# RemcoHoger/Space-Filling-Curves-for-Vision-Transformers

Measured on AMD Instinct MI355X. Metric: images/sec ViT-B/16 224px Hilbert-order training, higher is better.
Workload: dtype bf16; 1 GPU; vit_b16_224_hilbert: 224x224 Hilbert pixel order, 16x16-pixel tokens, batch 256/GPU, full train step (fwd+CE+bwd+clip+AdamW); global_batch=256, parallelism=dp1, hip_graph=False

## Files before the change

space-filling-curves-for-vision-transformers_amd/csrc/gemm8p.hip:

```cpp
#include "common_host.h"
#include "gemm_core.h"
#include <mutex>
#include <type_traits>
#include <unordered_map>

namespace sfcvit {
namespace {

using namespace gemm_core;

namespace p8 {

constexpr int T = 512, HALF = 16384, KTB = 65536, LDS_BYTES = 2 * KTB;
constexpr int LDS_TQ = LDS_BYTES, LDS_PATCH = LDS_TQ + 64, LDS_BIAS = LDS_PATCH + 8 * 2048, LDS_MAX = P8_LDS_MAX;
static_assert(LDS_BIAS == P8_LDS_BIAS, "dispatch.h prices the bias vector at this offset");
enum { RELU = P8_RELU, DROP = P8_DROP, RES = P8_RES, DACT = P8_DACT, CSUM = P8_CSUM, BITS = P8_BITS };

typedef const __attribute__((address_space(1))) void *gptr_t;
typedef __attribute__((address_space(3))) void *lptr_t;

template <int N> __device__ __forceinline__ void wait_vm() { asm volatile("s_waitcnt vmcnt(%0)" ::"n"(N) : "memory"); }
template <int N> __device__ __forceinline__ void wait_lgkm() {
    asm volatile("s_waitcnt lgkmcnt(%0)" ::"n"(N) : "memory");
    __builtin_amdgcn_sched_barrier(0);
}
__device__ __forceinline__ void bar() {
    __builtin_amdgcn_sched_barrier(0);
    __builtin_amdgcn_s_barrier();
    __builtin_amdgcn_sched_barrier(0);
}

struct Cursor {
    int tile, k0;
    const uint16_t *p;
};

struct StoreMap {
    int wa;
    int ra;
    long coff;
};

template <int MASK>
__device__ __forceinline__ void epilogue_math(const sfcvit_gemm_args &g, int m, int n, float (&v)[16], const float (&bv)[16],
                                              const u32x4 (&side)[2], uint32_t thresh, float keep_scale, float dact_scale,
                                              uint32_t rk_in0, uint32_t rk_in1, u32x4 &w0, u32x4 &w1) {
    if (!(MASK & DACT)) {
#pragma unroll
        for (int r = 0; r < 16; r++) v[r] += bv[r];
    }
    if (MASK & RELU) {
#pragma unroll
        for (int r = 0; r < 16; r++) v[r] = fmaxf(v[r], 0.f);
    }
    if (MASK & DROP) {
        const uint64_t row = uint64_t(m) + uint64_t(uint32_t(g.row_offset));
        const uint32_t rk = mix32(uint32_t(row) * 0x9E3779B1u + ((row >> 32) ? rk_in1 : rk_in0));
#pragma unroll
        for (int p = 0; p < 8; p++) {
            bool k0, k1;
            drop_keep2(rk, uint32_t(n >> 1) + p, thresh, k0, k1);
            v[2 * p] = k0 ? v[2 * p] * keep_scale : 0.f;
            v[2 * p + 1] = k1 ? v[2 * p + 1] * keep_scale : 0.f;
        }
    }
    if (MASK & RES) {
        float rv[16];
        unpack8f(side[0], rv);
        unpack8f(side[1], rv + 8);
#pragma unroll
        for (int r = 0; r < 16; r++) v[r] += rv[r];
    }
    if ((MASK & BITS) && (MASK & RELU)) {
        uint32_t bits = 0;
#pragma unroll
        for (int r = 0; r < 16; r++) bits |= uint32_t(v[r] > 0.f) << r;
        uint8_t *mp = static_cast<uint8_t *>(g.actmask) + size_t(m) * g.ld_actmask + (n >> 3);
        asm volatile("global_store_short %0, %1, off\n\ts_nop 1" ::"v"(mp), "v"(bits) : "memory");
    }
    if (MASK & DACT) {
        if (MASK & BITS) {
            const uint32_t bits = side[0][0];
#pragma unroll
            for (int r = 0; r < 16; r++) v[r] = (bits >> r & 1u) ? v[r] * dact_scale : 0.f;
        } else {
            float a[16];
            unpack8f(side[0], a);
            unpack8f(side[1], a + 8);
#pragma unroll
            for (int r = 0; r < 16; r++) v[r] = a[r] > 0.f ? v[r] * dact_scale : 0.f;
        }
    }
    w0 = u32x4{pack2bf(v[0], v[1]), pack2bf(v[2], v[3]), pack2bf(v[4], v[5]), pack2bf(v[6], v[7])};
    w1 = u32x4{pack2bf(v[8], v[9]), pack2bf(v[10], v[11]), pack2bf(v[12], v[13]), pack2bf(v[14], v[15])};
}

#define SFCVIT_XROW(a, b) "ds_write_b128 %[wa], " a "\n\tds_write_b128 %[wb], " b "\n\tds_read_b128 " a ", %[ra]\n\tds_read_b128 " b ", %[ra] offset:1024\n\t"
template <int NR>
__device__ __forceinline__ void patch_exchange(u32x4 (&w)[NR][2], const StoreMap &sm) {
    static_assert(NR >= 1 && NR <= 8, "rows per batch");
    const int wa = sm.wa, wb = sm.wa ^ 16, ra = sm.ra;
    if constexpr (NR == 8)
        asm volatile(SFCVIT_XROW("%0", "%1") SFCVIT_XROW("%2", "%3") SFCVIT_XROW("%4", "%5") SFCVIT_XROW("%6", "%7")
                     SFCVIT_XROW("%8", "%9") SFCVIT_XROW("%10", "%11") SFCVIT_XROW("%12", "%13") SFCVIT_XROW("%14", "%15") "s_waitcnt lgkmcnt(0)"
                     : "+v"(w[0][0]), "+v"(w[0][1]), "+v"(w[1][0]), "+v"(w[1][1]), "+v"(w[2][0]), "+v"(w[2][1]), "+v"(w[3][0]), "+v"(w[3][1]),
                       "+v"(w[4][0]), "+v"(w[4][1]), "+v"(w[5][0]), "+v"(w[5][1]), "+v"(w[6][0]), "+v"(w[6][1]), "+v"(w[7][0]), "+v"(w[7][1])
                     : [wa] "v"(wa), [wb] "v"(wb), [ra] "v"(ra) : "memory");
    else if constexpr (NR == 7)
        asm volatile(SFCVIT_XROW("%0", "%1") SFCVIT_XROW("%2", "%3") SFCVIT_XROW("%4", "%5") SFCVIT_XROW("%6", "%7")
                     SFCVIT_XROW("%8", "%9") SFCVIT_XROW("%10", "%11") SFCVIT_XROW("%12", "%13") "s_waitcnt lgkmcnt(0)"
                     : "+v"(w[0][0]), "+v"(w[0][1]), "+v"(w[1][0]), "+v"(w[1][1]), "+v"(w[2][0]), "+v"(w[2][1]), "+v"(w[3][0]), "+v"(w[3][1]),
                       "+v"(w[4][0]), "+v"(w[4][1]), "+v"(w[5][0]), "+v"(w[5][1]), "+v"(w[6][0]), "+v"(w[6][1])
                     : [wa] "v"(wa), [wb] "v"(wb), [ra] "v"(ra) : "memory");
    else if constexpr (NR == 6)
        asm volatile(SFCVIT_XROW("%0", "%1") SFCVIT_XROW("%2", "%3") SFCVIT_XROW("%4", "%5") SFCVIT_XROW("%6", "%7")
                     SFCVIT_XROW("%8", "%9") SFCVIT_XROW("%10", "%11") "s_waitcnt lgkmcnt(0)"
                     : "+v"(w[0][0]), "+v"(w[0][1]), "+v"(w[1][0]), "+v"(w[1][1]), "+v"(w[2][0]), "+v"(w[2][1]), "+v"(w[3][0]), "+v"(w[3][1]),
                       "+v"(w[4][0]), "+v"(w[4][1]), "+v"(w[5][0]), "+v"(w[5][1])
                     : [wa] "v"(wa), [wb] "v"(wb), [ra] "v"(ra) : "memory");
    else if constexpr (NR == 4)
        asm volatile(SFCVIT_XROW("%0", "%1") SFCVIT_XROW("%2", "%3") SFCVIT_XROW("%4", "%5") SFCVIT_XROW("%6", "%7") "s_waitcnt lgkmcnt(0)"
                     : "+v"(w[0][0]), "+v"(w[0][1]), "+v"(w[1][0]), "+v"(w[1][1]), "+v"(w[2][0]), "+v"(w[2][1]), "+v"(w[3][0]), "+v"(w[3][1])
                     : [wa] "v"(wa), [wb] "v"(wb), [ra] "v"(ra) : "memory");
    else
        static_assert(NR == 8, "patch_exchange: batch sizes 4, 6, 7, 8");
}
#undef SFCVIT_XROW

__device__ __forceinline__ void store_row_pair(const sfcvit_gemm_args &g, int m, int n, const StoreMap &sm, const u32x4 &w0, const u32x4 &w1) {
    uint16_t *c = static_cast<uint16_t *>(g.c) + size_t(m) * g.ldc + n + sm.coff;
    asm volatile("global_store_dwordx4 %0, %1, off sc0 sc1 nt\n\ts_nop 1" ::"v"(c), "v"(w0) : "memory");
    asm volatile("global_store_dwordx4 %0, %1, off sc0 sc1 nt\n\ts_nop 1" ::"v"(c + size_t(8) * g.ldc), "v"(w1) : "memory");
}


template <int NI, int MASK, bool P2 = false>
__global__ __launch_bounds__(T) void gemm8p_kernel(const sfcvit_gemm_args g, unsigned *__restrict__ counters, int stag_slots, int stag_ticks, int walk) {
    constexpr int BM = 32 * NI, GR = 16 * NI;
    extern __shared__ __attribute__((aligned(16))) char smem[];
    if (stag_ticks > 0) {
        const uint64_t until = __builtin_amdgcn_s_memrealtime() + uint64_t((blockIdx.x >> 3) % stag_slots) * uint64_t(stag_ticks);
        while (__builtin_amdgcn_s_memrealtime() < until) __builtin_amdgcn_s_sleep(8);
    }
    const int tid = threadIdx.x, lane = tid & 63, wid = __builtin_amdgcn_readfirstlane(tid >> 6), wr = wid >> 2, wc = wid & 3;
    const int q = lane >> 4, nl = lane & 15;
    const int K = g.K, NT = g.N / 256, ntiles = ((g.M + BM - 1) / BM) * NT, KT = K / 64, m_last = g.M - BM;
    const uint16_t *A = static_cast<const uint16_t *>(g.a);
    const uint16_t *B = static_cast<const uint16_t *>(g.b);
    const int G = gridDim.x, per_xcd = G >> 3, xcd = blockIdx.x & 7;
    int *const tq = reinterpret_cast<int *>(smem + LDS_TQ);
    auto tile_of = [&](unsigned l) __attribute__((always_inline)) {
        const long t = long(l / unsigned(per_xcd)) * G + xcd * per_xcd + int(l % unsigned(per_xcd));
        if (t >= ntiles) return -1;
        if (walk > 0 && walk < NT) {
            const unsigned MT = unsigned(ntiles / NT), full = unsigned(NT / walk) * MT * unsigned(walk), ut = unsigned(t);
            const unsigned wcur = ut < full ? unsigned(walk) : unsigned(NT % walk), base = ut < full ? (ut / (MT * walk)) * walk : unsigned(NT / walk) * walk;
            const unsigned tt = ut < full ? ut % (MT * walk) : ut - full;
            return int((tt / wcur) << 16 | (base + tt % wcur));
        }
        return int((unsigned(t) / unsigned(NT)) << 16 | (unsigned(t) % unsigned(NT)));
    };
    auto finish = [&]() __attribute__((always_inline)) {
        if (tid == 0) {
            const unsigned old = atomicAdd(counters + 8, 1u);
            if (old == unsigned(G) - 1u) {
#pragma unroll
                for (int i = 0; i < 9; i++) counters[i] = 0u;
            }
        }
    };
    if (tid == 0) {
        const unsigned l0 = atomicAdd(counters + xcd, 1u);
        tq[0] = tile_of(l0);
        const unsigned l1 = atomicAdd(counters + xcd, 1u);
        tq[1] = tile_of(l1);
    }
    const bool has_bias = !(MASK & DACT) && g.bias != nullptr;
    if (has_bias)
        for (int i = tid; i < g.N / 8; i += T)
            *reinterpret_cast<u32x4 *>(smem + LDS_BIAS + i * 16) = static_cast<const u32x4 *>(g.bias)[i];
    __syncthreads();

    int tile_cur = __builtin_amdgcn_readfirstlane(tq[0]);
    if (tile_cur < 0) { finish(); return; }
    unsigned drawn = 0;
    if (tid == 0) drawn = atomicAdd(counters + xcd, 1u);
    const int tile_first = tile_cur;
    int t = 0;

    const int r1 = 8 * wid + (lane >> 3);
    const int sc = (lane & 7) ^ ((r1 >> 1) & 7);
    const int w1 = (r1 < GR - 64) ? r1 : r1 - (NI == 7 ? 16 : 32);
    const int b_row = (r1 >> 5) * 64 + ((r1 & 15) >> 2) * 16 + ((r1 >> 4) & 1) * 4 + (r1 & 3);
    const uint32_t voffA0 = (uint32_t(r1) * uint32_t(g.lda) + sc * 8) * 2, voffA1 = (uint32_t(64 + w1) * uint32_t(g.lda) + sc * 8) * 2;
    const uint32_t voffB = (uint32_t(b_row) * uint32_t(g.ldb) + sc * 8) * 2;
    const size_t a_second = size_t(GR) * g.lda, b_second = size_t(128) * g.ldb, b_h1 = size_t(8) * g.ldb;

    auto cursor_at = [&](int seq, int tile, bool is_a) __attribute__((always_inline)) {
        Cursor c;
        c.tile = seq;
        c.k0 = 0;
        if (tile < 0) tile = tile_first;
        c.p = is_a ? A + size_t(min((tile >> 16) * BM, m_last)) * g.lda : B + size_t(tile & 0xFFFF) * 256 * g.ldb;
        return c;
    };
    const uint16_t *next_a = nullptr, *next_b = nullptr;
    auto set_next = [&](int seq) __attribute__((always_inline)) {
        const Cursor na = cursor_at(seq, __builtin_amdgcn_readfirstlane(tq[seq & 3]), true);
        const Cursor nb = cursor_at(seq, __builtin_amdgcn_readfirstlane(tq[seq & 3]), false);
        next_a = na.p;
        next_b = nb.p;
    };
    auto advance = [&](Cursor &c, bool is_a) __attribute__((always_inline)) {
        if (c.k0 + 64 == K) { c.tile++; c.k0 = 0; c.p = is_a ? next_a : next_b; }
        else { c.k0 += 64; c.p += 64; }
    };
    const int m0_wave = wid * 1024;
    auto dma16 = [&](const uint16_t *base, uint32_t voff, int lds) __attribute__((always_inline)) {
        asm volatile("s_mov_b32 m0, %2\n\ts_nop 0\n\tglobal_load_lds_dwordx4 %0, %1"
                     :
                     : "v"(voff), "s"(base), "s"(lds)
                     : "memory");
    };
    auto stage_a = [&](const Cursor &c, int buf, int h) __attribute__((always_inline)) {
        const int d = m0_wave + buf * KTB + h * HALF;
        const uint32_t vo = h ? voffA1 : voffA0;
        dma16(c.p, vo, d);
        dma16(c.p + a_second, vo, d + 8192);
    };
    auto stage_b = [&](const Cursor &c, int buf, int h) __attribute__((always_inline)) {
        const uint16_t *p = c.p + (h ? b_h1 : 0);
        const int d = m0_wave + buf * KTB + 2 * HALF + h * HALF;
        dma16(p, voffB, d);
        dma16(p + b_second, voffB, d + 8192);
    };

    const int o0 = nl * 128 + ((q ^ ((nl >> 1) & 7)) << 4);
    const int a_off0 = wr * 8192 + o0, a_off1 = wr * 8192 + (o0 ^ 64);
    const int b_off0 = 2 * HALF + wc * 4096 + o0, b_off1 = 2 * HALF + wc * 4096 + (o0 ^ 64);
    bf16x8 fa0[4][2], fa1[NI - 4][2], fb0[2][2], fb1[2][2];
    auto read_a0 = [&](int buf) __attribute__((always_inline)) {
#pragma unroll
        for (int i = 0; i < 4; i++) {
            fa0[i][0] = *reinterpret_cast<const bf16x8 *>(smem + a_off0 + buf * KTB + i * 2048);
            fa0[i][1] = *reinterpret_cast<const bf16x8 *>(smem + a_off1 + buf * KTB + i * 2048);
        }
    };
    auto read_a1 = [&](int buf) __attribute__((always_inline)) {
#pragma unroll
        for (int i = 0; i < NI - 4; i++) {
            fa1[i][0] = *reinterpret_cast<const bf16x8 *>(smem + a_off0 + buf * KTB + HALF + i * 2048);
            fa1[i][1] = *reinterpret_cast<const bf16x8 *>(smem + a_off1 + buf * KTB + HALF + i * 2048);
        }
    };
    auto read_b = [&](bf16x8 (&fb)[2][2], int buf, int sub) __attribute__((always_inline)) {
#pragma unroll
        for (int j = 0; j < 2; j++) {
            fb[j][0] = *reinterpret_cast<const bf16x8 *>(smem + b_off0 + buf * KTB + sub * HALF + j * 2048);
            fb[j][1] = *reinterpret_cast<const bf16x8 *>(smem + b_off1 + buf * KTB + sub * HALF + j * 2048);
        }
    };

    f32x4 acc[NI][4];
    auto zero_acc = [&]() __attribute__((always_inline)) {
#pragma unroll
        for (int i = 0; i < NI; i++)
#pragma unroll
            for (int j = 0; j < 4; j++) acc[i][j] = f32x4{0.f, 0.f, 0.f, 0.f};
    };
    auto mma0 = [&](const bf16x8 (&fb)[2][2], int bsub) __attribute__((always_inline)) {
        __builtin_amdgcn_s_setprio(1);
#pragma unroll
        for (int kk = 0; kk < 2; kk++)
#pragma unroll
            for (int i = 0; i < 4; i++)
#pragma unroll
                for (int j = 0; j < 2; j++)
                    acc[i][bsub * 2 + j] = __builtin_amdgcn_mfma_f32_16x16x32_bf16(fb[j][kk], fa0[i][kk], acc[i][bsub * 2 + j], 0, 0, 0);
        __builtin_amdgcn_s_setprio(0);
    };
    auto mma1 = [&](const bf16x8 (&fb)[2][2], int bsub) __attribute__((always_inline)) {
        __builtin_amdgcn_s_setprio(1);
#pragma unroll
        for (int kk = 0; kk < 2; kk++)
#pragma unroll
            for (int i = 0; i < NI - 4; i++)
#pragma unroll
                for (int j = 0; j < 2; j++)
                    acc[4 + i][bsub * 2 + j] = __builtin_amdgcn_mfma_f32_16x16x32_bf16(fb[j][kk], fa1[i][kk], acc[4 + i][bsub * 2 + j], 0, 0, 0);
        __builtin_amdgcn_s_setprio(0);
    };

    const uint32_t thresh = (MASK & DROP) ? drop_thresh(g.dropout_p) : 0u;
    const float keep_scale = (MASK & DROP) ? 1.f / (1.f - g.dropout_p) : 1.f;
    const uint32_t seed_e = (MASK & DROP) ? eff_seed(g.dropout_seed, g.seed_off) : 0u;
    const uint32_t rk_in0 = (MASK & DROP) ? mix32(seed_e) : 0u, rk_in1 = (MASK & DROP) ? mix32(seed_e ^ 0x7FEB352Du) : 0u;
    const float dact_scale = g.dact_scale != 0.f ? g.dact_scale : 1.f;
    auto draw = [&]() __attribute__((always_inline)) {
        if (tid == 0) {
            tq[(t + 2) & 3] = tile_of(drawn);
            drawn = atomicAdd(counters + xcd, 1u);
        }
    };
    auto epilogue = [&]() __attribute__((always_inline)) {
        const int tile = tile_cur;
        int te = tid;
        asm volatile("" : "+v"(te));
        const int le = te & 63, qe = le >> 4, ne = le & 15;
        StoreMap sm;
        {
            const int patch = LDS_PATCH + wid * 2048, r0 = le >> 3, ch = le & 7;
            sm.wa = patch + ne * 128 + (((2 * qe) ^ (ne & 7)) << 4);
            sm.ra = patch + r0 * 128 + ((ch ^ r0) << 4);
            sm.coff = long(r0 - ne) * g.ldc + (8 * ch - 16 * qe);
        }
        const int m_new = (tile >> 16) * BM;
        const int m0 = min(m_new, m_last) + wr * GR + ne, n0 = (tile & 0xFFFF) * 256 + wc * 64 + qe * 16;
        mfma_fence();
        float bv[16];
        if (has_bias) {
            const char *bp = smem + LDS_BIAS + n0 * 2;
            unpack8f(*reinterpret_cast<const u32x4 *>(bp), bv);
            unpack8f(*reinterpret_cast<const u32x4 *>(bp + 16), bv + 8);
        } else {
#pragma unroll
            for (int r = 0; r < 16; r++) bv[r] = 0.f;
        }
        const uint16_t *sp = (MASK & RES) ? static_cast<const uint16_t *>(g.residual) : static_cast<const uint16_t *>(g.aux_in);
        const size_t ld_side = (MASK & RES) ? size_t(g.ldr) : size_t(g.ldaux);
        float cs[16];
#pragma unroll
        for (int r = 0; r < 16; r++) cs[r] = 0.f;
        auto batch = [&](auto i0c, auto i1c) __attribute__((always_inline)) {
            constexpr int i0 = decltype(i0c)::value, i1 = decltype(i1c)::value;
            u32x4 side[i1 - i0][2];
            if ((MASK & DACT) && (MASK & BITS)) {
#pragma unroll
                for (int i = i0; i < i1; i++)
                    side[i - i0][0][0] = *reinterpret_cast<const uint16_t *>(static_cast<const uint8_t *>(g.actmask) +
                                                                             size_t(m0 + 16 * i) * g.ld_actmask + (n0 >> 3));
            } else if (MASK & (RES | DACT)) {
#pragma unroll
                for (int i = i0; i < i1; i++) {
                    const uint16_t *p = sp + size_t(m0 + 16 * i) * ld_side + n0;
                    side[i - i0][0] = *reinterpret_cast<const u32x4 *>(p);
                    side[i - i0][1] = *reinterpret_cast<const u32x4 *>(p + 8);
                }
            }
            u32x4 pk[i1 - i0][2];
            static_for<i0, i1>([&](auto ic) __attribute__((always_inline)) {
                constexpr int i = decltype(ic)::value;
                float v[16] = {acc[i][0][0], acc[i][0][1], acc[i][0][2], acc[i][0][3], acc[i][1][0], acc[i][1][1],
                               acc[i][1][2], acc[i][1][3], acc[i][2][0], acc[i][2][1], acc[i][2][2], acc[i][2][3],
                               acc[i][3][0], acc[i][3][1], acc[i][3][2], acc[i][3][3]};
                epilogue_math<MASK>(g, m0 + 16 * i, n0, v, bv, side[i - i0], thresh, keep_scale, dact_scale, rk_in0, rk_in1,
                                    pk[i - i0][0], pk[i - i0][1]);
                if (MASK & CSUM) {
                    const bool own = m0 + 16 * i >= m_new;
#pragma unroll
                    for (int r = 0; r < 16; r++) cs[r] += own ? v[r] : 0.f;
                }
            });
            patch_exchange<i1 - i0>(pk, sm);
            static_for<i0, i1>([&](auto ic) __attribute__((always_inline)) {
                constexpr int i = decltype(ic)::value;
                store_row_pair(g, m0 + 16 * i, n0, sm, pk[i - i0][0], pk[i - i0][1]);
            });
        };
        if constexpr (NI == 8 && ((MASK & (DROP | RES)) == (DROP | RES) || (MASK & (DACT | CSUM | BITS)) == (DACT | CSUM))) {
            batch(std::integral_constant<int, 0>{}, std::integral_constant<int, 4>{});
            batch(std::integral_constant<int, 4>{}, std::integral_constant<int, NI>{});
        } else {
            batch(std::integral_constant<int, 0>{}, std::integral_constant<int, NI>{});
        }
        if (MASK & CSUM) {
#pragma unroll
            for (int r = 0; r < 16; r++) cs[r] = row16_sum(cs[r]);
            if (ne == 0) {
                float *pp = static_cast<float *>(g.workspace) + size_t(2 * (tile >> 16) + wr) * g.N + n0;
#pragma unroll
                for (int r4 = 0; r4 < 4; r4++)
                    *reinterpret_cast<f32x4 *>(pp + 4 * r4) = f32x4{cs[4 * r4], cs[4 * r4 + 1], cs[4 * r4 + 2], cs[4 * r4 + 3]};
            }
        }
        zero_acc();
    };

    Cursor ca = cursor_at(0, tile_cur, true), cb = cursor_at(0, tile_cur, false);
    stage_b(cb, 0, 0); stage_a(ca, 0, 0); stage_a(ca, 0, 1); stage_b(cb, 0, 1);
    advance(ca, true);
    advance(cb, false);
    if (P2) {
        stage_b(cb, 1, 0); stage_a(ca, 1, 0); stage_b(cb, 1, 1);
        advance(cb, false);
        wait_vm<6>();
    } else {
        stage_b(cb, 1, 0); stage_a(ca, 1, 0); stage_a(ca, 1, 1); stage_b(cb, 1, 1);
        advance(ca, true);
        advance(cb, false);
        wait_vm<8>();
    }
    bar();
    if (wr == 1) bar();
    zero_acc();

    constexpr int NSTORE = 2 * NI + ((MASK & CSUM) ? 4 : 0) + (((MASK & BITS) && (MASK & RELU)) ? NI : 0);
    auto stage_next = [&](int buf) __attribute__((always_inline)) {
        stage_a(ca, buf, 1);
        advance(ca, true);
        stage_b(cb, buf, 1);
        advance(cb, false);
        __builtin_amdgcn_sched_barrier(0);
    };
    auto ktile = [&](int buf, bool first, bool last) __attribute__((always_inline)) {
        read_b(fb0, buf, 0);
        read_a0(buf);
        bar();
        wait_lgkm<0>();
        mma0(fb0, 0);
        bar();
        read_a1(buf);
        bar();
        wait_lgkm<0>();
        mma1(fb0, 0);
        if (first) set_next(t + 1);
        bar();
        read_b(fb1, buf, 1);
        stage_b(cb, buf, 0);
        bar();
        wait_lgkm<0>();
        mma1(fb1, 1);
        bar();
        stage_a(ca, buf, 0);
        if (first && t > 0) wait_vm<4 + NSTORE>();
        else wait_vm<4>();
        bar();
        mma0(fb1, 1);
        if (last) {
            if (wr == 0) {
                bar();
                draw();
            }
            stage_next(buf);
            epilogue();
            if (wr == 1) bar();
        } else {
            bar();
            stage_next(buf);
        }
    };
    auto ktile2 = [&](int buf, bool first, bool last) __attribute__((always_inline)) {
        read_b(fb0, buf, 0);
        read_b(fb1, buf, 1);
        read_a0(buf);
        stage_a(ca, buf ^ 1, 1);
        advance(ca, true);
        __builtin_amdgcn_sched_barrier(0);
        if (first && t > 0) wait_vm<8 + NSTORE>();
        else wait_vm<8>();
        wait_lgkm<0>();
        bar();
        mma0(fb0, 0);
        mma0(fb1, 1);
        if (first) set_next(t + 1);
        bar();
        read_a1(buf);
        stage_b(cb, buf, 0);
        stage_a(ca, buf, 0);
        stage_b(cb, buf, 1);
        advance(cb, false);
        __builtin_amdgcn_sched_barrier(0);
        if (first && t > 0) wait_vm<8 + NSTORE>();
        else wait_vm<8>();
        wait_lgkm<0>();
        bar();
        mma1(fb0, 0);
        mma1(fb1, 1);
        if (last) {
            if (wr == 0) {
                bar();
                draw();
            }
            epilogue();
            if (wr == 1) bar();
        } else {
            bar();
        }
    };
    int kt = 0;
    for (;;) {
        if (P2) ktile2(0, kt == 0, false);
        else ktile(0, kt == 0, false);
        kt += 2;
        const bool last = kt == KT;
        if (P2) ktile2(1, false, last);
        else ktile(1, false, last);
        if (last) {
            kt = 0;
            t++;
            tile_cur = __builtin_amdgcn_readfirstlane(tq[t & 3]);
            if (tile_cur < 0) break;
        }
    }
    if (wr == 0) bar();
    wait_vm<0>();
    finish();
}


template <bool P2>
__global__ __launch_bounds__(T) void gemm8p_km_kernel(const sfcvit_gemm_args g, int kt_per_split, int nsplits) {
    extern __shared__ __attribute__((aligned(16))) char smem[];
    const int tid = threadIdx.x, lane = tid & 63, wid = tid >> 6, wr = wid >> 2, wc = wid & 3;
    const int q4 = lane >> 4, nl = lane & 15;
    const int NT = g.N / 256, KT = g.K / 64;
    const int tiles = (g.M / 256) * NT;
    const int unit = (blockIdx.x & 7) * (gridDim.x >> 3) + (blockIdx.x >> 3);
    if (unit >= tiles * nsplits) return;
    const int tile = unit % tiles, z = unit / tiles;
    const int m0 = (tile / NT) * 256, n0 = (tile % NT) * 256;
    const int kt_beg = z * kt_per_split;
    const int nkt = min(kt_per_split, KT - kt_beg);
    const uint16_t *A = static_cast<const uint16_t *>(g.a) + size_t(kt_beg) * 64 * g.lda + m0;
    const uint16_t *B = static_cast<const uint16_t *>(g.b) + size_t(kt_beg) * 64 * g.ldb + n0;

    const int kr = 4 * wid + (lane >> 4);
    const int sw = (kr & 3) | (((kr >> 3) & 1) << 2);
    const int c16 = ((((lane & 15) >> 1) ^ sw) << 1) | (lane & 1);
    const size_t offA = size_t(kr) * g.lda + c16 * 8, offB = size_t(kr) * g.ldb + c16 * 8;
    const size_t a32 = size_t(32) * g.lda, b32 = size_t(32) * g.ldb, a64 = size_t(64) * g.lda, b64 = size_t(64) * g.ldb;
    char *const lds_piece = smem + tid * 16;
    const uint16_t *ca = A, *cb = B;
    int akt = 0, bkt = 0;
    auto advance_a = [&]() __attribute__((always_inline)) {
        if (++akt < nkt) ca += a64;
    };
    auto advance_b = [&]() __attribute__((always_inline)) {
        if (++bkt < nkt) cb += b64;
    };
    auto stage_a = [&](int buf, int h) __attribute__((always_inline)) {
        const uint16_t *p = ca + offA + h * 128;
        char *d = lds_piece + buf * KTB + h * HALF;
        __builtin_amdgcn_global_load_lds((gptr_t)p, (lptr_t)d, 16, 0, 0);
        __builtin_amdgcn_global_load_lds((gptr_t)(p + a32), (lptr_t)(d + 8192), 16, 0, 0);
    };
    auto stage_b = [&](int buf, int h) __attribute__((always_inline)) {
        const uint16_t *p = cb + offB + h * 128;
        char *d = lds_piece + buf * KTB + 2 * HALF + h * HALF;
        __builtin_amdgcn_global_load_lds((gptr_t)p, (lptr_t)d, 16, 0, 0);
        __builtin_amdgcn_global_load_lds((gptr_t)(p + b32), (lptr_t)(d + 8192), 16, 0, 0);
    };

    const int qq = nl >> 2, pp = nl & 3;
    const int lane_sw = qq | ((q4 & 1) << 2);
    const int row_off = (8 * q4 + qq) * 256 + 8 * pp;
    int a_addr[8], b_addr[4];
#pragma unroll
    for (int i = 0; i < 8; i++)
        a_addr[i] = (i >> 2) * HALF + row_off + (((wr * 4 + (i & 3)) ^ lane_sw) << 5);
#pragma unroll
    for (int j = 0; j < 4; j++)
        b_addr[j] = 2 * HALF + (j >> 1) * HALF + row_off + (((wc * 2 + (j & 1)) ^ lane_sw) << 5);
#define SFCVIT_TR(dst, addr, off) asm volatile("ds_read_b64_tr_b16 %0, %1 offset:" #off : "=v"(dst) : "v"(addr) : "memory")
    auto tr_frag2 = [&](bf16x8 (&f)[2], int addr) __attribute__((always_inline)) {
        bf16x4 l0, h0, l1, h1;
        SFCVIT_TR(l0, addr, 0);
        SFCVIT_TR(h0, addr, 1024);
        SFCVIT_TR(l1, addr, 8192);
        SFCVIT_TR(h1, addr, 9216);
        f[0] = __builtin_shufflevector(l0, h0, 0, 1, 2, 3, 4, 5, 6, 7);
        f[1] = __builtin_shufflevector(l1, h1, 0, 1, 2, 3, 4, 5, 6, 7);
    };
    bf16x8 fa0[4][2], fa1[4][2], fb0[2][2], fb1[2][2];
    auto read_a2 = [&](bf16x8 (&fa)[4][2], int sub, int i0) __attribute__((always_inline)) {
#pragma unroll
        for (int i = i0; i < i0 + 2; i++) tr_frag2(fa[i], a_addr[sub * 4 + i]);
    };
    auto read_b = [&](bf16x8 (&fb)[2][2], int sub) __attribute__((always_inline)) {
#pragma unroll
        for (int j = 0; j < 2; j++) tr_frag2(fb[j], b_addr[sub * 2 + j]);
    };
    auto flip = [&]() __attribute__((always_inline)) {
#pragma unroll
        for (int i = 0; i < 8; i++) a_addr[i] ^= KTB;
#pragma unroll
        for (int j = 0; j < 4; j++) b_addr[j] ^= KTB;
    };

    f32x4 acc[8][4];
#pragma unroll
    for (int i = 0; i < 8; i++)
#pragma unroll
        for (int j = 0; j < 4; j++) acc[i][j] = f32x4{0.f, 0.f, 0.f, 0.f};
    auto mma = [&](const bf16x8 (&fa)[4][2], const bf16x8 (&fb)[2][2], int asub, int bsub) __attribute__((always_inline)) {
        __builtin_amdgcn_s_setprio(1);
#pragma unroll
        for (int kk = 0; kk < 2; kk++)
#pragma unroll
            for (int i = 0; i < 4; i++)
#pragma unroll
                for (int j = 0; j < 2; j++)
                    acc[asub * 4 + i][bsub * 2 + j] =
                        __builtin_amdgcn_mfma_f32_16x16x32_bf16(fb[j][kk], fa[i][kk], acc[asub * 4 + i][bsub * 2 + j], 0, 0, 0);
        __builtin_amdgcn_s_setprio(0);
    };

    if (P2) {
        stage_b(0, 0); stage_a(0, 0); stage_a(0, 1); stage_b(0, 1);
        advance_a();
        advance_b();
        stage_b(1, 0); stage_a(1, 0); stage_b(1, 1);
        advance_b();
        wait_vm<6>();
        bar();
        if (wr == 1) bar();
        auto ktile2 = [&](int buf) __attribute__((always_inline)) {
            read_b(fb0, 0);
            read_b(fb1, 1);
            read_a2(fa0, 0, 0);
            read_a2(fa0, 0, 2);
            stage_a(buf ^ 1, 1);
            advance_a();
            wait_vm<8>();
            wait_lgkm<0>();
            bar();
            mma(fa0, fb0, 0, 0);
            mma(fa0, fb1, 0, 1);
            bar();
            read_a2(fa1, 1, 0);
            read_a2(fa1, 1, 2);
            stage_b(buf, 0);
            stage_a(buf, 0);
            stage_b(buf, 1);
            advance_b();
            wait_vm<8>();
            wait_lgkm<0>();
            bar();
            mma(fa1, fb0, 1, 0);
            mma(fa1, fb1, 1, 1);
            bar();
            flip();
        };
        for (int k = 0; k < nkt; k += 2) {
            ktile2(0);
            ktile2(1);
        }
    } else {
        stage_b(0, 0); stage_a(0, 0); stage_a(0, 1); stage_b(0, 1);
        advance_a();
// ... 144 lines not shown
```

Baseline: 8260 images/s.

## Trim register pressure and scalar bookkeeping in persistent GEMM kernel

Drops the per-cursor tile and k0 counters and replaces the K-boundary test in advance with a wrap flag computed in the outer loop. Lane-dependent constants are recomputed after the epilogue, and empty asm barriers keep leading dimensions and scheduling values in SGPRs, to lower VGPR pressure in the heavy DROP|RES variant. Accumulator zeroing is overlapped with the LDS patch exchange by splitting the wait out of patch_exchange. The aim is to avoid spills and cut scalar and vector overhead in the main loop, at the cost of fragile compiler-steering asm and some recomputation.

```diff
diff --git a/space-filling-curves-for-vision-transformers_amd/csrc/gemm8p.hip b/space-filling-curves-for-vision-transformers_amd/csrc/gemm8p.hip
--- a/space-filling-curves-for-vision-transformers_amd/csrc/gemm8p.hip
+++ b/space-filling-curves-for-vision-transformers_amd/csrc/gemm8p.hip
@@ -31,7 +31,6 @@
 }
 
 struct Cursor {
-    int tile, k0;
     const uint16_t *p;
 };
 
@@ -42,7 +41,7 @@
 };
 
 template <int MASK>
-__device__ __forceinline__ void epilogue_math(const sfcvit_gemm_args &g, int m, int n, float (&v)[16], const float (&bv)[16],
+__device__ __forceinline__ void epilogue_math(const sfcvit_gemm_args &g, int ld_bits, int m, int n, float (&v)[16], const float (&bv)[16],
                                               const u32x4 (&side)[2], uint32_t thresh, float keep_scale, float dact_scale,
                                               uint32_t rk_in0, uint32_t rk_in1, u32x4 &w0, u32x4 &w1) {
     if (!(MASK & DACT)) {
@@ -75,7 +74,7 @@
         uint32_t bits = 0;
 #pragma unroll
         for (int r = 0; r < 16; r++) bits |= uint32_t(v[r] > 0.f) << r;
-        uint8_t *mp = static_cast<uint8_t *>(g.actmask) + size_t(m) * g.ld_actmask + (n >> 3);
+        uint8_t *mp = static_cast<uint8_t *>(g.actmask) + size_t(m) * ld_bits + (n >> 3);
         asm volatile("global_store_short %0, %1, off\n\ts_nop 1" ::"v"(mp), "v"(bits) : "memory");
     }
     if (MASK & DACT) {
@@ -96,72 +95,102 @@
 }
 
 #define SFCVIT_XROW(a, b) "ds_write_b128 %[wa], " a "\n\tds_write_b128 %[wb], " b "\n\tds_read_b128 " a ", %[ra]\n\tds_read_b128 " b ", %[ra] offset:1024\n\t"
+#define SFCVIT_W4 "+v"(w[0][0]), "+v"(w[0][1]), "+v"(w[1][0]), "+v"(w[1][1]), "+v"(w[2][0]), "+v"(w[2][1]), "+v"(w[3][0]), "+v"(w[3][1])
+#define SFCVIT_W6 SFCVIT_W4, "+v"(w[4][0]), "+v"(w[4][1]), "+v"(w[5][0]), "+v"(w[5][1])
+#define SFCVIT_W7 SFCVIT_W6, "+v"(w[6][0]), "+v"(w[6][1])
+#define SFCVIT_W8 SFCVIT_W7, "+v"(w[7][0]), "+v"(w[7][1])
+#define SFCVIT_X4 SFCVIT_XROW("%0", "%1") SFCVIT_XROW("%2", "%3") SFCVIT_XROW("%4", "%5") SFCVIT_XROW("%6", "%7")
+#define SFCVIT_X6 SFCVIT_X4 SFCVIT_XROW("%8", "%9") SFCVIT_XROW("%10", "%11")
+#define SFCVIT_X7 SFCVIT_X6 SFCVIT_XROW("%12", "%13")
+#define SFCVIT_X8 SFCVIT_X7 SFCVIT_XROW("%14", "%15")
 template <int NR>
 __device__ __forceinline__ void patch_exchange(u32x4 (&w)[NR][2], const StoreMap &sm) {
-    static_assert(NR >= 1 && NR <= 8, "rows per batch");
+    static_assert(NR == 4 || NR == 6 || NR == 7 || NR == 8, "patch_exchange: batch sizes 4, 6, 7, 8");
     const int wa = sm.wa, wb = sm.wa ^ 16, ra = sm.ra;
-    if constexpr (NR == 8)
-        asm volatile(SFCVIT_XROW("%0", "%1") SFCVIT_XROW("%2", "%3") SFCVIT_XROW("%4", "%5") SFCVIT_XROW("%6", "%7")
-                     SFCVIT_XROW("%8", "%9") SFCVIT_XROW("%10", "%11") SFCVIT_XROW("%12", "%13") SFCVIT_XROW("%14", "%15") "s_waitcnt lgkmcnt(0)"
-                     : "+v"(w[0][0]), "+v"(w[0][1]), "+v"(w[1][0]), "+v"(w[1][1]), "+v"(w[2][0]), "+v"(w[2][1]), "+v"(w[3][0]), "+v"(w[3][1]),
-                       "+v"(w[4][0]), "+v"(w[4][1]), "+v"(w[5][0]), "+v"(w[5][1]), "+v"(w[6][0]), "+v"(w[6][1]), "+v"(w[7][0]), "+v"(w[7][1])
-                     : [wa] "v"(wa), [wb] "v"(wb), [ra] "v"(ra) : "memory");
-    else if constexpr (NR == 7)
-        asm volatile(SFCVIT_XROW("%0", "%1") SFCVIT_XROW("%2", "%3") SFCVIT_XROW("%4", "%5") SFCVIT_XROW("%6", "%7")
-                     SFCVIT_XROW("%8", "%9") SFCVIT_XROW("%10", "%11") SFCVIT_XROW("%12", "%13") "s_waitcnt lgkmcnt(0)"
-                     : "+v"(w[0][0]), "+v"(w[0][1]), "+v"(w[1][0]), "+v"(w[1][1]), "+v"(w[2][0]), "+v"(w[2][1]), "+v"(w[3][0]), "+v"(w[3][1]),
-                       "+v"(w[4][0]), "+v"(w[4][1]), "+v"(w[5][0]), "+v"(w[5][1]), "+v"(w[6][0]), "+v"(w[6][1])
-                     : [wa] "v"(wa), [wb] "v"(wb), [ra] "v"(ra) : "memory");
-    else if constexpr (NR == 6)
-        asm volatile(SFCVIT_XROW("%0", "%1") SFCVIT_XROW("%2", "%3") SFCVIT_XROW("%4", "%5") SFCVIT_XROW("%6", "%7")
-                     SFCVIT_XROW("%8", "%9") SFCVIT_XROW("%10", "%11") "s_waitcnt lgkmcnt(0)"
-                     : "+v"(w[0][0]), "+v"(w[0][1]), "+v"(w[1][0]), "+v"(w[1][1]), "+v"(w[2][0]), "+v"(w[2][1]), "+v"(w[3][0]), "+v"(w[3][1]),
-                       "+v"(w[4][0]), "+v"(w[4][1]), "+v"(w[5][0]), "+v"(w[5][1])
-                     : [wa] "v"(wa), [wb] "v"(wb), [ra] "v"(ra) : "memory");
-    else if constexpr (NR == 4)
-        asm volatile(SFCVIT_XROW("%0", "%1") SFCVIT_XROW("%2", "%3") SFCVIT_XROW("%4", "%5") SFCVIT_XROW("%6", "%7") "s_waitcnt lgkmcnt(0)"
-                     : "+v"(w[0][0]), "+v"(w[0][1]), "+v"(w[1][0]), "+v"(w[1][1]), "+v"(w[2][0]), "+v"(w[2][1]), "+v"(w[3][0]), "+v"(w[3][1])
-                     : [wa] "v"(wa), [wb] "v"(wb), [ra] "v"(ra) : "memory");
-    else
-        static_assert(NR == 8, "patch_exchange: batch sizes 4, 6, 7, 8");
-}
+    if constexpr (NR == 8) asm volatile(SFCVIT_X8 : SFCVIT_W8 : [wa] "v"(wa), [wb] "v"(wb), [ra] "v"(ra) : "memory");
+    else if constexpr (NR == 7) asm volatile(SFCVIT_X7 : SFCVIT_W7 : [wa] "v"(wa), [wb] "v"(wb), [ra] "v"(ra) : "memory");
+    else if constexpr (NR == 6) asm volatile(SFCVIT_X6 : SFCVIT_W6 : [wa] "v"(wa), [wb] "v"(wb), [ra] "v"(ra) : "memory");
+    else asm volatile(SFCVIT_X4 : SFCVIT_W4 : [wa] "v"(wa), [wb] "v"(wb), [ra] "v"(ra) : "memory");
+}
+template <int NR>
+__device__ __forceinline__ void patch_wait(u32x4 (&w)[NR][2]) {
+    if constexpr (NR == 8) asm volatile("s_waitcnt lgkmcnt(0)" : SFCVIT_W8 : : "memory");
+    else if constexpr (NR == 7) asm volatile("s_waitcnt lgkmcnt(0)" : SFCVIT_W7 : : "memory");
+    else if constexpr (NR == 6) asm volatile("s_waitcnt lgkmcnt(0)" : SFCVIT_W6 : : "memory");
+    else asm volatile("s_waitcnt lgkmcnt(0)" : SFCVIT_W4 : : "memory");
+}
+#undef SFCVIT_X8
+#undef SFCVIT_X7
+#undef SFCVIT_X6
+#undef SFCVIT_X4
+#undef SFCVIT_W8
+#undef SFCVIT_W7
+#undef SFCVIT_W6
+#undef SFCVIT_W4
 #undef SFCVIT_XROW
 
-__device__ __forceinline__ void store_row_pair(const sfcvit_gemm_args &g, int m, int n, const StoreMap &sm, const u32x4 &w0, const u32x4 &w1) {
-    uint16_t *c = static_cast<uint16_t *>(g.c) + size_t(m) * g.ldc + n + sm.coff;
+typedef float f32x2 __attribute__((ext_vector_type(2)));
+__device__ __forceinline__ void clear_quad(f32x4 &a) {
+    f32x2 lo, hi;
+    asm volatile("v_mov_b64 %0, 0\n\tv_mov_b64 %1, 0" : "=v"(lo), "=v"(hi));
+    a = __builtin_shufflevector(lo, hi, 0, 1, 2, 3);
+}
+
+__device__ __forceinline__ void store_row_pair(const sfcvit_gemm_args &g, int ldc, int m, int n, const StoreMap &sm, const u32x4 &w0, const u32x4 &w1) {
+    uint16_t *c = static_cast<uint16_t *>(g.c) + size_t(m) * ldc + n + sm.coff;
     asm volatile("global_store_dwordx4 %0, %1, off sc0 sc1 nt\n\ts_nop 1" ::"v"(c), "v"(w0) : "memory");
-    asm volatile("global_store_dwordx4 %0, %1, off sc0 sc1 nt\n\ts_nop 1" ::"v"(c + size_t(8) * g.ldc), "v"(w1) : "memory");
+    asm volatile("global_store_dwordx4 %0, %1, off sc0 sc1 nt\n\ts_nop 1" ::"v"(c + size_t(8) * ldc), "v"(w1) : "memory");
 }
 
 
 template <int NI, int MASK, bool P2 = false>
 __global__ __launch_bounds__(T) void gemm8p_kernel(const sfcvit_gemm_args g, unsigned *__restrict__ counters, int stag_slots, int stag_ticks, int walk) {
     constexpr int BM = 32 * NI, GR = 16 * NI;
+    constexpr bool tight = NI == 8 && (MASK & (DROP | RES)) == (DROP | RES);
+    constexpr bool lean_draw = tight || (!P2 && (MASK & DROP) != 0);
     extern __shared__ __attribute__((aligned(16))) char smem[];
     if (stag_ticks > 0) {
         const uint64_t until = __builtin_amdgcn_s_memrealtime() + uint64_t((blockIdx.x >> 3) % stag_slots) * uint64_t(stag_ticks);
         while (__builtin_amdgcn_s_memrealtime() < until) __builtin_amdgcn_s_sleep(8);
     }
-    const int tid = threadIdx.x, lane = tid & 63, wid = __builtin_amdgcn_readfirstlane(tid >> 6), wr = wid >> 2, wc = wid & 3;
-    const int q = lane >> 4, nl = lane & 15;
-    const int K = g.K, NT = g.N / 256, ntiles = ((g.M + BM - 1) / BM) * NT, KT = K / 64, m_last = g.M - BM;
+    const int tid = threadIdx.x, wid = __builtin_amdgcn_readfirstlane(tid >> 6), wr = wid >> 2, wc = wid & 3;
+    auto is_thread0 = [&]() __attribute__((always_inline)) {
+        int x = tid;
+        asm volatile("" : "+v"(x));
+        return x == 0;
+    };
+    auto group = [&]() __attribute__((always_inline)) {
+        int x = wr;
+        asm volatile("" : "+s"(x));
+        return x;
+    };
+    const int KT = g.K / 64, m_last = g.M - BM;
     const uint16_t *A = static_cast<const uint16_t *>(g.a);
     const uint16_t *B = static_cast<const uint16_t *>(g.b);
-    const int G = gridDim.x, per_xcd = G >> 3, xcd = blockIdx.x & 7;
+    const int G = gridDim.x, xcd = blockIdx.x & 7;
     int *const tq = reinterpret_cast<int *>(smem + LDS_TQ);
     auto tile_of = [&](unsigned l) __attribute__((always_inline)) {
-        const long t = long(l / unsigned(per_xcd)) * G + xcd * per_xcd + int(l % unsigned(per_xcd));
-        if (t >= ntiles) return -1;
-        if (walk > 0 && walk < NT) {
-            const unsigned MT = unsigned(ntiles / NT), full = unsigned(NT / walk) * MT * unsigned(walk), ut = unsigned(t);
-            const unsigned wcur = ut < full ? unsigned(walk) : unsigned(NT % walk), base = ut < full ? (ut / (MT * walk)) * walk : unsigned(NT / walk) * walk;
-            const unsigned tt = ut < full ? ut % (MT * walk) : ut - full;
+        unsigned gu = unsigned(G), nu = unsigned(g.N), wk = unsigned(walk), mt = unsigned(m_last);
+        if constexpr (lean_draw) asm volatile("" : "+s"(gu), "+s"(nu), "+s"(wk), "+s"(mt));
+        const unsigned px = gu >> 3, nt = nu / 256u;
+        const unsigned ntiles = ((mt + unsigned(2 * BM - 1)) / unsigned(BM)) * nt;
+        const long t = long(l / px) * long(gu) + long(unsigned(xcd) * px + l % px);
+        if (t >= long(ntiles)) return -1;
+        if (wk > 0u && wk < nt) {
+            const unsigned MT = ntiles / nt, full = (nt / wk) * MT * wk, ut = unsigned(t);
+            const unsigned wcur = ut < full ? wk : nt % wk, base = ut < full ? (ut / (MT * wk)) * wk : (nt / wk) * wk;
+            const unsigned tt = ut < full ? ut % (MT * wk) : ut - full;
             return int((tt / wcur) << 16 | (base + tt % wcur));
         }
-        return int((unsigned(t) / unsigned(NT)) << 16 | (unsigned(t) % unsigned(NT)));
+        return int((unsigned(t) / nt) << 16 | (unsigned(t) % nt));
+    };
+    auto queue = [&]() __attribute__((always_inline)) {
+        int x = xcd;
+        asm volatile("" : "+s"(x));
+        return counters + x;
     };
     auto finish = [&]() __attribute__((always_inline)) {
-        if (tid == 0) {
+        if (is_thread0()) {
             const unsigned old = atomicAdd(counters + 8, 1u);
             if (old == unsigned(G) - 1u) {
 #pragma unroll
@@ -170,9 +199,9 @@
         }
     };
     if (tid == 0) {
-        const unsigned l0 = atomicAdd(counters + xcd, 1u);
+        const unsigned l0 = atomicAdd(queue(), 1u);
         tq[0] = tile_of(l0);
-        const unsigned l1 = atomicAdd(counters + xcd, 1u);
+        const unsigned l1 = atomicAdd(queue(), 1u);
         tq[1] = tile_of(l1);
     }
     const bool has_bias = !(MASK & DACT) && g.bias != nullptr;
@@ -184,39 +213,57 @@
     int tile_cur = __builtin_amdgcn_readfirstlane(tq[0]);
     if (tile_cur < 0) { finish(); return; }
     unsigned drawn = 0;
-    if (tid == 0) drawn = atomicAdd(counters + xcd, 1u);
-    const int tile_first = tile_cur;
+    if (tid == 0) drawn = atomicAdd(queue(), 1u);
     int t = 0;
 
-    const int r1 = 8 * wid + (lane >> 3);
-    const int sc = (lane & 7) ^ ((r1 >> 1) & 7);
-    const int w1 = (r1 < GR - 64) ? r1 : r1 - (NI == 7 ? 16 : 32);
-    const int b_row = (r1 >> 5) * 64 + ((r1 & 15) >> 2) * 16 + ((r1 >> 4) & 1) * 4 + (r1 & 3);
-    const uint32_t voffA0 = (uint32_t(r1) * uint32_t(g.lda) + sc * 8) * 2, voffA1 = (uint32_t(64 + w1) * uint32_t(g.lda) + sc * 8) * 2;
-    const uint32_t voffB = (uint32_t(b_row) * uint32_t(g.ldb) + sc * 8) * 2;
-    const size_t a_second = size_t(GR) * g.lda, b_second = size_t(128) * g.ldb, b_h1 = size_t(8) * g.ldb;
-
-    auto cursor_at = [&](int seq, int tile, bool is_a) __attribute__((always_inline)) {
+    uint32_t voffA0, voffA1, voffB;
+    int a_off0, a_off1, b_off0, b_off1;
+    auto lane_consts = [&]() __attribute__((always_inline)) {
+        int tl = tid;
+        if constexpr (tight) asm volatile("" : "+v"(tl));
+        const int ll = tl & 63, ql = ll >> 4, nll = ll & 15;
+        const int r1 = 8 * wid + (ll >> 3);
+        const int sc = (ll & 7) ^ ((r1 >> 1) & 7);
+        const int w1 = (r1 < GR - 64) ? r1 : r1 - (NI == 7 ? 16 : 32);
+        const int b_row = (r1 >> 5) * 64 + ((r1 & 15) >> 2) * 16 + ((r1 >> 4) & 1) * 4 + (r1 & 3);
+        voffA0 = (uint32_t(r1) * uint32_t(g.lda) + sc * 8) * 2;
+        voffA1 = (uint32_t(64 + w1) * uint32_t(g.lda) + sc * 8) * 2;
+        voffB = (uint32_t(b_row) * uint32_t(g.ldb) + sc * 8) * 2;
+        const int o0 = nll * 128 + ((ql ^ ((nll >> 1) & 7)) << 4);
+        a_off0 = wr * 8192 + o0;
+        a_off1 = wr * 8192 + (o0 ^ 64);
+        b_off0 = 2 * HALF + wc * 4096 + o0;
+        b_off1 = 2 * HALF + wc * 4096 + (o0 ^ 64);
+    };
+    lane_consts();
+    auto ld_bytes = [&](int ld) __attribute__((always_inline)) {
+        uint32_t x = uint32_t(ld);
+        if constexpr (tight) asm volatile("" : "+s"(x));
+        return x * 2u;
+    };
+    auto a_second = [&]() __attribute__((always_inline)) { return uint32_t(GR) * ld_bytes(g.lda); };
+    auto b_second = [&]() __attribute__((always_inline)) { return 128u * ld_bytes(g.ldb); };
+    auto b_h1 = [&]() __attribute__((always_inline)) { return 8u * ld_bytes(g.ldb); };
+
+    auto cursor_at = [&](int tile, bool is_a) __attribute__((always_inline)) {
         Cursor c;
-        c.tile = seq;
-        c.k0 = 0;
-        if (tile < 0) tile = tile_first;
+        if (tile < 0) tile = tile_cur;
         c.p = is_a ? A + size_t(min((tile >> 16) * BM, m_last)) * g.lda : B + size_t(tile & 0xFFFF) * 256 * g.ldb;
         return c;
     };
     const uint16_t *next_a = nullptr, *next_b = nullptr;
     auto set_next = [&](int seq) __attribute__((always_inline)) {
-        const Cursor na = cursor_at(seq, __builtin_amdgcn_readfirstlane(tq[seq & 3]), true);
-        const Cursor nb = cursor_at(seq, __builtin_amdgcn_readfirstlane(tq[seq & 3]), false);
+        const Cursor na = cursor_at(__builtin_amdgcn_readfirstlane(tq[seq & 3]), true);
+        const Cursor nb = cursor_at(__builtin_amdgcn_readfirstlane(tq[seq & 3]), false);
         next_a = na.p;
         next_b = nb.p;
     };
-    auto advance = [&](Cursor &c, bool is_a) __attribute__((always_inline)) {
-        if (c.k0 + 64 == K) { c.tile++; c.k0 = 0; c.p = is_a ? next_a : next_b; }
-        else { c.k0 += 64; c.p += 64; }
+    auto advance = [&](Cursor &c, bool is_a, bool wrap) __attribute__((always_inline)) {
+        if (wrap) c.p = is_a ? next_a : next_b;
+        else c.p += 64;
     };
     const int m0_wave = wid * 1024;
-    auto dma16 = [&](const uint16_t *base, uint32_t voff, int lds) __attribute__((always_inline)) {
+    auto dma16 = [&](const char *base, uint32_t voff, int lds) __attribute__((always_inline)) {
         asm volatile("s_mov_b32 m0, %2\n\ts_nop 0\n\tglobal_load_lds_dwordx4 %0, %1"
                      :
                      : "v"(voff), "s"(base), "s"(lds)
@@ -225,39 +272,46 @@
     auto stage_a = [&](const Cursor &c, int buf, int h) __attribute__((always_inline)) {
         const int d = m0_wave + buf * KTB + h * HALF;
         const uint32_t vo = h ? voffA1 : voffA0;
-        dma16(c.p, vo, d);
-        dma16(c.p + a_second, vo, d + 8192);
+        const char *p = reinterpret_cast<const char *>(c.p);
+        dma16(p, vo, d);
+        dma16(p + a_second(), vo, d + 8192);
     };
     auto stage_b = [&](const Cursor &c, int buf, int h) __attribute__((always_inline)) {
-        const uint16_t *p = c.p + (h ? b_h1 : 0);
+        const char *p = reinterpret_cast<const char *>(c.p) + (h ? b_h1() : 0u);
         const int d = m0_wave + buf * KTB + 2 * HALF + h * HALF;
         dma16(p, voffB, d);
-        dma16(p + b_second, voffB, d + 8192);
-    };
-
-    const int o0 = nl * 128 + ((q ^ ((nl >> 1) & 7)) << 4);
-    const int a_off0 = wr * 8192 + o0, a_off1 = wr * 8192 + (o0 ^ 64);
-    const int b_off0 = 2 * HALF + wc * 4096 + o0, b_off1 = 2 * HALF + wc * 4096 + (o0 ^ 64);
+        dma16(p + b_second(), voffB, d + 8192);
+    };
+
     bf16x8 fa0[4][2], fa1[NI - 4][2], fb0[2][2], fb1[2][2];
+    auto frag_at = [&](int off0, int off1, int kk, int add) __attribute__((always_inline)) {
+        if constexpr (tight && !P2) {
+            int x = off0;
+            asm volatile("" : "+v"(x));
+            return (kk ? x ^ 64 : x) + add;
+        } else {
+            return (kk ? off1 : off0) + add;
+        }
+    };
     auto read_a0 = [&](int buf) __attribute__((always_inline)) {
 #pragma unroll
         for (int i = 0; i < 4; i++) {
-            fa0[i][0] = *reinterpret_cast<const bf16x8 *>(smem + a_off0 + buf * KTB + i * 2048);
-            fa0[i][1] = *reinterpret_cast<const bf16x8 *>(smem + a_off1 + buf * KTB + i * 2048);
+            fa0[i][0] = *reinterpret_cast<const bf16x8 *>(smem + frag_at(a_off0, a_off1, 0, buf * KTB) + i * 2048);
+            fa0[i][1] = *reinterpret_cast<const bf16x8 *>(smem + frag_at(a_off0, a_off1, 1, buf * KTB) + i * 2048);
         }
     };
     auto read_a1 = [&](int buf) __attribute__((always_inline)) {
 #pragma unroll
         for (int i = 0; i < NI - 4; i++) {
-            fa1[i][0] = *reinterpret_cast<const bf16x8 *>(smem + a_off0 + buf * KTB + HALF + i * 2048);
-            fa1[i][1] = *reinterpret_cast<const bf16x8 *>(smem + a_off1 + buf * KTB + HALF + i * 2048);
+            fa1[i][0] = *reinterpret_cast<const bf16x8 *>(smem + frag_at(a_off0, a_off1, 0, buf * KTB) + HALF + i * 2048);
+            fa1[i][1] = *reinterpret_cast<const bf16x8 *>(smem + frag_at(a_off0, a_off1, 1, buf * KTB) + HALF + i * 2048);
         }
     };
     auto read_b = [&](bf16x8 (&fb)[2][2], int buf, int sub) __attribute__((always_inline)) {
 #pragma unroll
         for (int j = 0; j < 2; j++) {
-            fb[j][0] = *reinterpret_cast<const bf16x8 *>(smem + b_off0 + buf * KTB + sub * HALF + j * 2048);
-            fb[j][1] = *reinterpret_cast<const bf16x8 *>(smem + b_off1 + buf * KTB + sub * HALF + j * 2048);
+            fb[j][0] = *reinterpret_cast<const bf16x8 *>(smem + frag_at(b_off0, b_off1, 0, buf * KTB) + sub * HALF + j * 2048);
+            fb[j][1] = *reinterpret_cast<const bf16x8 *>(smem + frag_at(b_off0, b_off1, 1, buf * KTB) + sub * HALF + j * 2048);
         }
     };
 
@@ -293,13 +347,13 @@
 
     const uint32_t thresh = (MASK & DROP) ? drop_thresh(g.dropout_p) : 0u;
     const float keep_scale = (MASK & DROP) ? 1.f / (1.f - g.dropout_p) : 1.f;
-    const uint32_t seed_e = (MASK & DROP) ? eff_seed(g.dropout_seed, g.seed_off) : 0u;
+    const uint32_t seed_e = (MASK & DROP) ? __builtin_amdgcn_readfirstlane(eff_seed(g.dropout_seed, g.seed_off)) : 0u;
     const uint32_t rk_in0 = (MASK & DROP) ? mix32(seed_e) : 0u, rk_in1 = (MASK & DROP) ? mix32(seed_e ^ 0x7FEB352Du) : 0u;
     const float dact_scale = g.dact_scale != 0.f ? g.dact_scale : 1.f;
     auto draw = [&]() __attribute__((always_inline)) {
-        if (tid == 0) {
+        if (is_thread0()) {
             tq[(t + 2) & 3] = tile_of(drawn);
-            drawn = atomicAdd(counters + xcd, 1u);
+            drawn = atomicAdd(queue(), 1u);
         }
     };
     auto epilogue = [&]() __attribute__((always_inline)) {
@@ -307,12 +361,16 @@
         int te = tid;
         asm volatile("" : "+v"(te));
         const int le = te & 63, qe = le >> 4, ne = le & 15;
+        int ldc = g.ldc, ld_side_i = (MASK & RES) ? g.ldr : g.ldaux, ld_bits = g.ld_actmask;
+        asm volatile("" : "+s"(ldc));
+        if constexpr ((MASK & (RES | DACT)) != 0 && !((MASK & DACT) && (MASK & BITS))) asm volatile("" : "+s"(ld_side_i));
+        if constexpr ((MASK & BITS) != 0) asm volatile("" : "+s"(ld_bits));
         StoreMap sm;
         {
             const int patch = LDS_PATCH + wid * 2048, r0 = le >> 3, ch = le & 7;
             sm.wa = patch + ne * 128 + (((2 * qe) ^ (ne & 7)) << 4);
             sm.ra = patch + r0 * 128 + ((ch ^ r0) << 4);
-            sm.coff = long(r0 - ne) * g.ldc + (8 * ch - 16 * qe);
+            sm.coff = long(r0 - ne) * ldc + (8 * ch - 16 * qe);
         }
         const int m_new = (tile >> 16) * BM;
         const int m0 = min(m_new, m_last) + wr * GR + ne, n0 = (tile & 0xFFFF) * 256 + wc * 64 + qe * 16;
@@ -327,18 +385,20 @@
             for (int r = 0; r < 16; r++) bv[r] = 0.f;
         }
         const uint16_t *sp = (MASK & RES) ? static_cast<const uint16_t *>(g.residual) : static_cast<const uint16_t *>(g.aux_in);
-        const size_t ld_side = (MASK & RES) ? size_t(g.ldr) : size_t(g.ldaux);
+        const size_t ld_side = size_t(ld_side_i);
         float cs[16];
 #pragma unroll
         for (int r = 0; r < 16; r++) cs[r] = 0.f;
+        constexpr bool two_batches = NI == 8 && ((MASK & (DROP | RES)) == (DROP | RES) || (MASK & (DACT | CSUM | BITS)) == (DACT | CSUM));
         auto batch = [&](auto i0c, auto i1c) __attribute__((always_inline)) {
             constexpr int i0 = decltype(i0c)::value, i1 = decltype(i1c)::value;
+            constexpr bool final_batch = i1 == NI;
             u32x4 side[i1 - i0][2];
             if ((MASK & DACT) && (MASK & BITS)) {
 #pragma unroll
                 for (int i = i0; i < i1; i++)
                     side[i - i0][0][0] = *reinterpret_cast<const uint16_t *>(static_cast<const uint8_t *>(g.actmask) +
-                                                                             size_t(m0 + 16 * i) * g.ld_actmask + (n0 >> 3));
+                                                                             size_t(m0 + 16 * i) * ld_bits + (n0 >> 3));
             } else if (MASK & (RES | DACT)) {
 #pragma unroll
                 for (int i = i0; i < i1; i++) {
@@ -353,21 +413,33 @@
                 float v[16] = {acc[i][0][0], acc[i][0][1], acc[i][0][2], acc[i][0][3], acc[i][1][0], acc[i][1][1],
                                acc[i][1][2], acc[i][1][3], acc[i][2][0], acc[i][2][1], acc[i][2][2], acc[i][2][3],
                                acc[i][3][0], acc[i][3][1], acc[i][3][2], acc[i][3][3]};
-                epilogue_math<MASK>(g, m0 + 16 * i, n0, v, bv, side[i - i0], thresh, keep_scale, dact_scale, rk_in0, rk_in1,
+                epilogue_math<MASK>(g, ld_bits, m0 + 16 * i, n0, v, bv, side[i - i0], thresh, keep_scale, dact_scale, rk_in0, rk_in1,
                                     pk[i - i0][0], pk[i - i0][1]);
                 if (MASK & CSUM) {
                     const bool own = m0 + 16 * i >= m_new;
 #pragma unroll
                     for (int r = 0; r < 16; r++) cs[r] += own ? v[r] : 0.f;
                 }
+                if constexpr (two_batches && i + 1 < NI)
+                    asm volatile("" : "+v"(pk[i - i0][0]), "+v"(pk[i - i0][1]), "+v"(acc[i + 1][0]), "+v"(acc[i + 1][1]), "+v"(acc[i + 1][2]), "+v"(acc[i + 1][3]));
             });
             patch_exchange<i1 - i0>(pk, sm);
+            if constexpr (final_batch) {
+                static_for<0, NI>([&](auto ic) __attribute__((always_inline)) {
+                    constexpr int i = decltype(ic)::value;
+                    clear_quad(acc[i][0]);
+                    clear_quad(acc[i][1]);
+                    clear_quad(acc[i][2]);
+                    clear_quad(acc[i][3]);
+                });
+            }
+            patch_wait<i1 - i0>(pk);
             static_for<i0, i1>([&](auto ic) __attribute__((always_inline)) {
                 constexpr int i = decltype(ic)::value;
-                store_row_pair(g, m0 + 16 * i, n0, sm, pk[i - i0][0], pk[i - i0][1]);
+                store_row_pair(g, ldc, m0 + 16 * i, n0, sm, pk[i - i0][0], pk[i - i0][1]);
             });
         };
-        if constexpr (NI == 8 && ((MASK & (DROP | RES)) == (DROP | RES) || (MASK & (DACT | CSUM | BITS)) == (DACT | CSUM))) {
+        if constexpr (two_batches) {
             batch(std::integral_constant<int, 0>{}, std::integral_constant<int, 4>{});
             batch(std::integral_constant<int, 4>{}, std::integral_constant<int, NI>{});
         } else {
@@ -383,21 +455,20 @@
                     *reinterpret_cast<f32x4 *>(pp + 4 * r4) = f32x4{cs[4 * r4], cs[4 * r4 + 1], cs[4 * r4 + 2], cs[4 * r4 + 3]};
             }
         }
-        zero_acc();
-    };
-
-    Cursor ca = cursor_at(0, tile_cur, true), cb = cursor_at(0, tile_cur, false);
+    };
+
+    Cursor ca = cursor_at(tile_cur, true), cb = cursor_at(tile_cur, false);
     stage_b(cb, 0, 0); stage_a(ca, 0, 0); stage_a(ca, 0, 1); stage_b(cb, 0, 1);
-    advance(ca, true);
-    advance(cb, false);
+    advance(ca, true, false);
+    advance(cb, false, false);
     if (P2) {
         stage_b(cb, 1, 0); stage_a(ca, 1, 0); stage_b(cb, 1, 1);
-        advance(cb, false);
+        advance(cb, false, false);
         wait_vm<6>();
     } else {
         stage_b(cb, 1, 0); stage_a(ca, 1, 0); stage_a(ca, 1, 1); stage_b(cb, 1, 1);
-        advance(ca, true);
-        advance(cb, false);
+        advance(ca, true, false);
+        advance(cb, false, false);
         wait_vm<8>();
     }
     bar();
@@ -405,14 +476,14 @@
     zero_acc();
 
     constexpr int NSTORE = 2 * NI + ((MASK & CSUM) ? 4 : 0) + (((MASK & BITS) && (MASK & RELU)) ? NI : 0);
-    auto stage_next = [&](int buf) __attribute__((always_inline)) {
+    auto stage_next = [&](int buf, bool wrap) __attribute__((always_inline)) {
         stage_a(ca, buf, 1);
-        advance(ca, true);
+        advance(ca, true, wrap);
         stage_b(cb, buf, 1);
-        advance(cb, false);
+        advance(cb, false, wrap);
         __builtin_amdgcn_sched_barrier(0);
     };
-    auto ktile = [&](int buf, bool first, bool last) __attribute__((always_inline)) {
+    auto ktile = [&](int buf, bool first, bool last, bool wrap) __attribute__((always_inline)) {
         read_b(fb0, buf, 0);
         read_a0(buf);
         bar();
@@ -437,24 +508,25 @@
         bar();
         mma0(fb1, 1);
         if (last) {
-            if (wr == 0) {
+            if (group() == 0) {
                 bar();
                 draw();
             }
-            stage_next(buf);
+            stage_next(buf, wrap);
             epilogue();
-            if (wr == 1) bar();
+            if constexpr (tight) lane_consts();
+            if (group() == 1) bar();
         } else {
             bar();
-            stage_next(buf);
-        }
-    };
-    auto ktile2 = [&](int buf, bool first, bool last) __attribute__((always_inline)) {
+            stage_next(buf, wrap);
+        }
+    };
+    auto ktile2 = [&](int buf, bool first, bool last, bool wrap_a, bool wrap_b) __attribute__((always_inline)) {
         read_b(fb0, buf, 0);
         read_b(fb1, buf, 1);
         read_a0(buf);
         stage_a(ca, buf ^ 1, 1);
-        advance(ca, true);
+        advance(ca, true, wrap_a);
         __builtin_amdgcn_sched_barrier(0);
         if (first && t > 0) wait_vm<8 + NSTORE>();
         else wait_vm<8>();
@@ -468,7 +540,7 @@
         stage_b(cb, buf, 0);
         stage_a(ca, buf, 0);
         stage_b(cb, buf, 1);
-        advance(cb, false);
+        advance(cb, false, wrap_b);
         __builtin_amdgcn_sched_barrier(0);
         if (first && t > 0) wait_vm<8 + NSTORE>();
         else wait_vm<8>();
@@ -477,24 +549,25 @@
         mma1(fb0, 0);
         mma1(fb1, 1);
         if (last) {
-            if (wr == 0) {
+            if (group() == 0) {
                 bar();
                 draw();
             }
             epilogue();
-            if (wr == 1) bar();
+            if constexpr (tight) lane_consts();
+            if (group() == 1) bar();
         } else {
             bar();
         }
     };
     int kt = 0;
     for (;;) {
-        if (P2) ktile2(0, kt == 0, false);
-        else ktile(0, kt == 0, false);
+        if (P2) ktile2(0, kt == 0, false, kt + 2 == KT, false);
+        else ktile(0, kt == 0, false, false);
         kt += 2;
-        const bool last = kt == KT;
-        if (P2) ktile2(1, false, last);
-        else ktile(1, false, last);
+        const bool last = kt == KT, wrap = kt + 2 == KT;
+        if (P2) ktile2(1, false, last, false, wrap);
+        else ktile(1, false, last, wrap);
         if (last) {
             kt = 0;
             t++;
```

New measurement: 8306 images/s (median of 6 runs). Within noise of the previous version (+0.6%).
